# darksim33/Pyneapple

Measured on AMD Instinct MI355X. Metric: voxels/sec (pixelwise triexp LM & 250-bin NNLS) at 1/2/4/8 MI355X, higher is better.
Workload: dtype f64

## Files before the change

### pyneapple_amd/csrc/pnx_api.hip

```cpp
#include <hip/hip_runtime.h>

#include <cmath>
#include <cstdarg>
#include <cstdio>
#include <cstring>
#include <algorithm>
#include <atomic>
#include <chrono>
#include <condition_variable>
#include <cstdlib>
#include <functional>
#include <mutex>
#include <string>
#include <thread>
#include <vector>

#include "pnx_curvefit_f32_kernel.hpp"
#include "pnx_curvefit_kernel.hpp"
#include "pnx_grid.hpp"
#include "pnx_grid_args.hpp"
#include "pnx_grid_class.hpp"
#include "pnx_grid_posterior.hpp"
#include "pnx_grid_marginal.hpp"
#include "pnx_grid_mrf.hpp"
// ... 109 lines not shown

static void touch_pages(void *p, size_t bytes) {
    if (!p || !bytes) return;
    volatile char *c = (volatile char *)p;
    const uintptr_t a = (uintptr_t)p;
    c[0] = 0;
    for (size_t off = (4096 - (a & 4095)) & 4095; off < bytes; off += 4096) c[off] = 0;
}

int env_int(const char *name, int dflt, int lo, int hi) {
    const char *e = getenv(name);
    if (!e) return dflt;
    const long v = atol(e);
    return v < lo ? lo : (v > hi ? hi : (int)v);
}
const char *dev_getenv(const char *name) {
    static const bool enabled = [] {
        const char *e = getenv("PNX_ENABLE_TEST_HOOKS");
        return e && e[0] == '1' && e[1] == 0;
    }();
    return enabled ? getenv(name) : nullptr;
}
int dev_env_int(const char *name, int dflt, int lo, int hi) { return dev_getenv(name) ? env_int(name, dflt, lo, hi) : dflt; }

static std::atomic<int> g_host_calls(0);
struct HostCallGuard {
    int in_flight;
    HostCallGuard() : in_flight(g_host_calls.fetch_add(1) + 1) {}
    ~HostCallGuard() { g_host_calls.fetch_sub(1); }
    int touchers() const { return getenv("PNX_HOST_TOUCHERS") ? env_int("PNX_HOST_TOUCHERS", 2, 0, 8) : (in_flight >= 3 ? 0 : (in_flight == 2 ? 1 : 2)); }
    int out_threads() const { return getenv("PNX_STREAM_OUT_THREADS") ? env_int("PNX_STREAM_OUT_THREADS", 2, 1, 4) : (in_flight >= 4 ? 1 : 2); }
};

struct Carver {
    char *base = nullptr;
    size_t off = 0;
    void *take(size_t bytes) {
        void *p = base ? base + off : nullptr;
        off += (bytes + 255) & ~(size_t)255;
        return p;
    }
};

static int model_n_params(int model) {
    switch (model) {
    case PNX_MODEL_MONO: return 2;
    case PNX_MODEL_BI_REDUCED: return 3;
    case PNX_MODEL_BI_S0: return 4;
    case PNX_MODEL_BI_FULL: return 4;
    case PNX_MODEL_TRI_REDUCED: return 5;
    case PNX_MODEL_TRI_S0: return 6;
    case PNX_MODEL_TRI_FULL: return 6;
    }
    return -1;
}

typedef int (*launch_fn)(int, int, const CurvefitArgs *, int, void *);
static launch_fn g_launch[7] = {pnx_launch_curvefit_m0, pnx_launch_curvefit_m1, pnx_launch_curvefit_m2,
                                pnx_launch_curvefit_m3, pnx_launch_curvefit_m4, pnx_launch_curvefit_m5,
                                pnx_launch_curvefit_m6};

struct StreamLaunch {
    StreamCtl *ctl = nullptr;
    unsigned int *host_flags = nullptr;
    int granule_shift = 0;
    unsigned int spins = 0;
    int phase = 0;
};

static int curvefit_device(const pnx_curvefit_opts *o, int64_t n_vox, const double *b, const double *y_d,
                           const double *p0, const double *lo, const double *hi, const double *fixed, double *popt_d,
                           double *pcov_d, int8_t *status_d, int32_t *nfev_d, double *cost_d, DeviceInfo *dev,
                           hipStream_t stream, const StreamLaunch *sl = nullptr, const int32_t *order = nullptr) {
    CurvefitArgs a;
    memset(&a, 0, sizeof(a));
    if (sl) {
        a.ctl = sl->ctl;
        a.host_flags = sl->host_flags;
        a.granule_shift = sl->granule_shift;
        a.stream_spins = sl->spins;
        a.phase = sl->phase;
    }
    a.team = dev_env_int("PNX_CF_TEAM", 1, 0, 1);
    a.order = sl ? nullptr : order;
    a.y = y_d;
    a.popt = popt_d;
    a.pcov = pcov_d;
    a.status = status_d;
    a.nfev = nfev_d;
    a.cost = cost_d;
    a.n_vox = n_vox;
    a.n_b = o->n_b;
    a.per_voxel = o->per_voxel_p0_bounds;
    a.fixed_per_voxel = o->fixed_per_voxel;
    a.max_nfev = o->max_nfev > 0 ? o->max_nfev : 100 * o->n_free;
    a.n_fixed = o->n_fixed;
    a.t1_mode = o->t1_mode;
    a.tr = o->tr;
    a.tm = o->tm;
    a.ftol = o->ftol;
    a.xtol = o->xtol;
    a.gtol = o->gtol;
    for (int k = 0; k < o->n_free; ++k) a.free_idx[k] = o->free_idx[k];
    for (int k = 0; k < o->n_fixed; ++k) a.fixed_idx[k] = o->fixed_idx[k];
    for (int i = 0; i < o->n_b; ++i) a.b[i] = b[i];
    a.absolute_sigma = o->absolute_sigma != 0;
    a.use_sigma = o->sigma != nullptr;
    if (o->sigma)
        for (int i = 0; i < o->n_b; ++i) a.w[i] = 1.0 / o->sigma[i];
    if (o->per_voxel_p0_bounds) {
        a.p0 = p0;
        a.lo = lo;
        a.hi = hi;
    } else {
        for (int k = 0; k < o->n_free; ++k) {
            a.p0s[k] = p0[k];
            a.los[k] = lo[k];
            a.his[k] = hi[k];
        }
    }
    if (o->n_fixed) {
        if (o->fixed_per_voxel)
            a.fixed = fixed;
        else
            for (int k = 0; k < o->n_fixed; ++k) a.fixeds[k] = fixed[k];
    }
    if (a.phase != 2) {
        a.queue = next_queue(dev);
        PNX_HIP(hipMemsetAsync(a.queue, 0, sizeof(unsigned long long), stream));
    }
    return g_launch[o->model](o->n_free, o->jac_mode, &a, dev->cus, (void *)stream);
}

static int check_curvefit_opts(const pnx_curvefit_opts *o) {
    if (!o) return set_error(PNX_ERR_INVALID, "opts is NULL");
    int n_all = model_n_params(o->model);
    if (n_all < 0) return set_error(PNX_ERR_INVALID, "unknown model %d", o->model);
    if (o->t1_mode < 0 || o->t1_mode > 2) return set_error(PNX_ERR_INVALID, "t1_mode %d", o->t1_mode);
    if (o->t1_mode) n_all += 1;
    if (o->n_b < 1 || o->n_b > PNX_MAX_BVALUES) return set_error(PNX_ERR_INVALID, "n_b=%d out of range [1,%d]", o->n_b, PNX_MAX_BVALUES);
    if (o->n_free < 1 || o->n_fixed < 0 || o->n_free + o->n_fixed != n_all)
        return set_error(PNX_ERR_INVALID, "n_free=%d + n_fixed=%d != %d parameters of model %d", o->n_free, o->n_fixed, n_all, o->model);
    bool seen[PNX_MAX_PARAMS] = {false};
    for (int k = 0; k < o->n_free; ++k) {
        const int j = o->free_idx[k];
        if (j < 0 || j >= n_all || seen[j] || (k && j <= o->free_idx[k - 1]))
            return set_error(PNX_ERR_INVALID, "free_idx must be ascending, unique positions in [0,%d)", n_all);
        seen[j] = true;
    }
    for (int k = 0; k < o->n_fixed; ++k) {
        const int j = o->fixed_idx[k];
        if (j < 0 || j >= n_all || seen[j]) return set_error(PNX_ERR_INVALID, "fixed_idx overlaps free_idx or is out of range");
        seen[j] = true;
    }
    if (o->jac_mode != PNX_JAC_FD && o->jac_mode != PNX_JAC_ANALYTIC) return set_error(PNX_ERR_INVALID, "jac_mode %d", o->jac_mode);
    if (o->jac_mode == PNX_JAC_FD && o->n_fixed)
        return set_error(PNX_ERR_UNSUPPORTED,
                         "finite-difference Jacobian with fixed parameters: the reference uses the analytic Jacobian "
                         "there (curvefit.py:274-288); pass PNX_JAC_ANALYTIC");
    if (!(o->ftol >= 0) || !(o->xtol >= 0) || !(o->gtol >= 0)) return set_error(PNX_ERR_INVALID, "tolerances must be >= 0");
    return PNX_OK;
}

}

using namespace pnx;
// ... 2872 lines not shown
```

### pyneapple_amd/csrc/pnx_curvefit_kernel.hpp

```cpp
#pragma once
#include <hip/hip_runtime.h>
#include <stdint.h>

#include "pnx_trf_math.hpp"

namespace pnx {

constexpr int kWave = 64;
constexpr int kMaxB = 128;
constexpr int kMaxP = 8;
#ifdef PNX_ROW_BLK
template <int N> constexpr int row_blk() { return PNX_ROW_BLK; }
#else
template <int N> constexpr int row_blk() { return N >= 7 ? 2 : (N >= 5 ? 4 : 8); }
#endif
constexpr double kEps = TrfTraits<double>::eps;
constexpr double kSqrtEps = 1.4901161193847656e-08;
template <bool B> struct BoolC {
    static constexpr bool value = B;
};
typedef __attribute__((address_space(3))) void lds_void;

struct StreamCtl {
    unsigned long long ready;
    unsigned int abort;
    unsigned int timed_out;
    unsigned int done[1];
};

struct CurvefitArgs {
    const double *y;
    const double *p0;
    const double *lo;
    const double *hi;
    const double *fixed;
    double *popt;
    double *pcov;
    int8_t *status;
    int32_t *nfev;
    double *cost;
    unsigned long long *queue;
    const int32_t *order;
    StreamCtl *ctl;
    unsigned int *host_flags;
    int granule_shift;
    unsigned int stream_spins;
    int phase;
    int team;
    long long n_vox;
    int n_b;
    int per_voxel;
    int fixed_per_voxel;
    int max_nfev;
    int n_fixed;
    int t1_mode;
    double tr, tm;
    double ftol, xtol, gtol;
    double p0s[kMaxP], los[kMaxP], his[kMaxP], fixeds[kMaxP];
    int free_idx[kMaxP];
    int fixed_idx[kMaxP];
    int use_sigma;
    int absolute_sigma;
    double b[kMaxB];
    double w[kMaxB];
};

template <int MODEL> struct Model;

template <> struct Model<0> {
    static constexpr int NALL = 2, NC = 1;
    __device__ static constexpr int dpos(int c) { return 1; }
    __device__ static double signal(const double *p, const double *E) { return p[0] * E[0]; }
    __device__ static void jac(const double *p, const double *E, double x, double *r) {
        r[0] = E[0];
        r[1] = -x * p[0] * E[0];
    }
};
template <> struct Model<1> {
    static constexpr int NALL = 3, NC = 2;
    __device__ static constexpr int dpos(int c) { return c == 0 ? 1 : 2; }
    __device__ static double signal(const double *p, const double *E) { return p[0] * E[0] + (1 - p[0]) * E[1]; }
    __device__ static void jac(const double *p, const double *E, double x, double *r) {
        r[0] = E[0] - E[1];
        r[1] = -x * p[0] * E[0];
        r[2] = -x * (1 - p[0]) * E[1];
    }
};
template <> struct Model<2> {
    static constexpr int NALL = 4, NC = 2;
    __device__ static constexpr int dpos(int c) { return c == 0 ? 1 : 2; }
    __device__ static double signal(const double *p, const double *E) {
        return p[3] * (p[0] * E[0] + (1 - p[0]) * E[1]);
    }
    __device__ static void jac(const double *p, const double *E, double x, double *r) {
        r[0] = p[3] * (E[0] - E[1]);
        r[1] = -x * p[3] * p[0] * E[0];
        r[2] = -x * p[3] * (1 - p[0]) * E[1];
        r[3] = p[0] * E[0] + (1 - p[0]) * E[1];
    }
};
template <> struct Model<3> {
    static constexpr int NALL = 4, NC = 2;
    __device__ static constexpr int dpos(int c) { return c == 0 ? 1 : 3; }
    __device__ static double signal(const double *p, const double *E) { return p[0] * E[0] + p[2] * E[1]; }
    __device__ static void jac(const double *p, const double *E, double x, double *r) {
        r[0] = E[0];
        r[1] = -x * p[0] * E[0];
        r[2] = E[1];
        r[3] = -x * p[2] * E[1];
    }
};
template <> struct Model<4> {
    static constexpr int NALL = 5, NC = 3;
    __device__ static constexpr int dpos(int c) { return c == 0 ? 1 : (c == 1 ? 3 : 4); }
    __device__ static double signal(const double *p, const double *E) {
        return p[0] * E[0] + p[2] * E[1] + (1 - p[0] - p[2]) * E[2];
    }
    __device__ static void jac(const double *p, const double *E, double x, double *r) {
        const double f3 = 1 - p[0] - p[2];
        r[0] = E[0] - E[2];
        r[1] = -x * p[0] * E[0];
        r[2] = E[1] - E[2];
        r[3] = -x * p[2] * E[1];
        r[4] = -x * f3 * E[2];
    }
};
template <> struct Model<5> {
    static constexpr int NALL = 6, NC = 3;
    __device__ static constexpr int dpos(int c) { return c == 0 ? 1 : (c == 1 ? 3 : 4); }
    __device__ static double signal(const double *p, const double *E) {
        return p[5] * (p[0] * E[0] + p[2] * E[1] + (1 - p[0] - p[2]) * E[2]);
    }
    __device__ static void jac(const double *p, const double *E, double x, double *r) {
        const double f3 = 1 - p[0] - p[2], S0 = p[5];
        r[0] = S0 * (E[0] - E[2]);
        r[1] = -x * S0 * p[0] * E[0];
        r[2] = S0 * (E[1] - E[2]);
        r[3] = -x * S0 * p[2] * E[1];
        r[4] = -x * S0 * f3 * E[2];
        r[5] = p[0] * E[0] + p[2] * E[1] + f3 * E[2];
    }
};
template <> struct Model<6> {
    static constexpr int NALL = 6, NC = 3;
    __device__ static constexpr int dpos(int c) { return c == 0 ? 1 : (c == 1 ? 3 : 5); }
    __device__ static double signal(const double *p, const double *E) {
        return p[0] * E[0] + p[2] * E[1] + p[4] * E[2];
    }
    __device__ static void jac(const double *p, const double *E, double x, double *r) {
        r[0] = E[0];
        r[1] = -x * p[0] * E[0];
        r[2] = E[1];
        r[3] = -x * p[2] * E[1];
        r[4] = E[2];
        r[5] = -x * p[4] * E[2];
    }
};

template <int MODEL> __host__ __device__ constexpr int colperm(int k) {
    constexpr int P[7][6] = {{0, 1, 2, 3, 4, 5}, {2, 0, 1, 3, 4, 5}, {2, 0, 1, 3, 4, 5}, {3, 1, 2, 0, 4, 5},
                             {4, 3, 0, 2, 1, 5}, {4, 3, 0, 2, 1, 5}, {5, 3, 1, 4, 2, 0}};
    return P[MODEL][k];
}

template <int MODEL> __device__ constexpr int comp_of_param(int j) {
    for (int c = 0; c < Model<MODEL>::NC; ++c)
        if (Model<MODEL>::dpos(c) == j) return c;
    return -1;
}

#ifndef PNX_CF_FAST_EXP
#define PNX_CF_FAST_EXP 1
#endif
#ifndef PNX_CF_HINTS
#define PNX_CF_HINTS 1
#endif
#if PNX_CF_HINTS
#define PNX_LIKELY(x) __builtin_expect(!!(x), 1)
#else
#define PNX_LIKELY(x) (x)
#endif
__device__ inline double exp_fast(double x) {
#if PNX_CF_FAST_EXP
    const double k = __builtin_rint(x * 1.4426950408889634);
    double r = fma(k, -0.6931471805599453, x);
    r = fma(k, -2.3190468138462996e-17, r);
    const double r2 = r * r;
    double qe = 2.7630903490112654e-07;
    qe = fma(qe, r2, 2.480149103909504e-05);
    qe = fma(qe, r2, 0.0013888888945916382);
    qe = fma(qe, r2, 0.041666666666519754);
    qe = fma(qe, r2, 0.5000000000000012);
    double qo = 2.502232256764614e-08;
    qo = fma(qo, r2, 2.755751454582531e-06);
    qo = fma(qo, r2, 0.00019841269589115522);
    qo = fma(qo, r2, 0.008333333333455043);
    qo = fma(qo, r2, 0.16666666666666477);
    const double q = fma(r, qo, qe);
    return ldexp(fma(r, fma(r, q, 1.0), 1.0), __double2int_rz(k));
#else
    return exp(x);
#endif
}

__device__ inline double lane_bcast(double v, int src) {
    const unsigned long long u = __builtin_bit_cast(unsigned long long, v);
    const unsigned int lo = __builtin_amdgcn_readlane((int)(unsigned int)u, src), hi = __builtin_amdgcn_readlane((int)(unsigned int)(u >> 32), src);
    return __builtin_bit_cast(double, ((unsigned long long)hi << 32) | lo);
}

enum LaneState : int { ST_IDLE = 0, ST_INIT = 1, ST_RUN = 2, ST_FINAL = 3 };

template <int N> struct Park {
    static constexpr int NR = N * (N + 1) / 2;
    static constexpr bool kParkV = (N <= 5);
    static constexpr int NV = kParkV ? N * N : 0;
    __host__ __device__ static constexpr int per_wave(int tile_rows) { return kWave * (tile_rows + NR + NV); }
    __host__ __device__ static constexpr int per_wave_f64(int n_b) { return kWave * (((n_b + 1) & ~1) + NR + NV); }
};

#ifndef PNX_CF_WAVES_PER_SIMD
#define PNX_CF_WAVES_PER_SIMD 1
#endif
#ifndef PNX_CF_BLOCK_WAVES
#define PNX_CF_BLOCK_WAVES 4
#endif
template <int MODEL, int N, bool FD, bool PV, bool T1, bool STREAM = false>
__global__ void __launch_bounds__(64 * PNX_CF_BLOCK_WAVES, PNX_CF_WAVES_PER_SIMD) curvefit_kernel(const CurvefitArgs A) {
    using M = Model<MODEL>;
    using PK = Park<N>;
    constexpr int NALL = M::NALL;
    constexpr int NP = NALL + (T1 ? 1 : 0);
    constexpr int NC = M::NC;
    constexpr bool HASFIXED = (N != NP);
    static_assert(!(FD && HASFIXED), "finite-difference mode is only built without fixed parameters");
    auto CP = [](int k) constexpr { return (HASFIXED || k >= NALL) ? k : colperm<MODEL>(k); };

    extern __shared__ double smem[];
    const int n_b = A.n_b;
    double *bsh = smem;
    const int lane = threadIdx.x & (kWave - 1);
    const int wave = threadIdx.x / kWave;
    const bool use_w = A.use_sigma != 0;
    const double *wsh = smem + kMaxB;
    double *ytile = smem + (use_w ? 2 * kMaxB : kMaxB) + (size_t)wave * PK::per_wave_f64(n_b);
    double *ysh = ytile + 2 * lane;
    double *rpark = ytile + (size_t)((n_b + 1) & ~1) * kWave + lane;
    double *vpark = rpark + (size_t)PK::NR * kWave;
    for (int i = threadIdx.x; i < n_b; i += blockDim.x) bsh[i] = A.b[i];
    if (use_w)
        for (int i = threadIdx.x; i < n_b; i += blockDim.x) smem[kMaxB + i] = A.w[i];
    double bmax = 0;
    for (int i = 0; i < n_b; ++i) {
        const double ab = fabs(A.b[i]);
        bmax = (ab < INFINITY) ? fmax(bmax, ab) : INFINITY;
    }
    __syncthreads();
    const bool dma_ok = ((reinterpret_cast<uintptr_t>(A.y) & 7) == 0);

    int state = ST_IDLE;
    long long vox = -1;
    unsigned long long ready_seen = 0;
    int pub = 0;
    auto publish = [&](bool all) {
        const int n_gran = (int)((A.n_vox + (1ll << A.granule_shift) - 1) >> A.granule_shift);
        int upto = pub;
        while (upto < n_gran && (all || !__ballot(state != ST_IDLE && (vox >> A.granule_shift) <= upto))) ++upto;
        if (upto == pub) return;
        __builtin_amdgcn_fence(__ATOMIC_RELEASE, "");
        const unsigned int n_waves = gridDim.x * (blockDim.x / kWave);
        if ((threadIdx.x & (kWave - 1)) == __ffsll((unsigned long long)__ballot(1)) - 1) {
            for (int g = pub; g < upto; ++g) {
                const unsigned int old = __hip_atomic_fetch_add(&A.ctl->done[g], 1u, __ATOMIC_ACQ_REL, __HIP_MEMORY_SCOPE_SYSTEM);
                if (old + 1 == n_waves) __hip_atomic_store(&A.host_flags[g], 1u, __ATOMIC_RELEASE, __HIP_MEMORY_SCOPE_SYSTEM);
            }
        }
        pub = upto;
    };
    double x[N], lb[N], ub[N];
    double pfull[NP];
    double g[N];
    double s[N], uf[N], R2[N][N], d[N], g_h[N];
    double Vreg[PK::kParkV ? 1 : N][PK::kParkV ? 1 : N];
    double smax = 0, smin = 0, theta = 0;
    double cost = 0, Delta = 0, alpha = 0;
    int nfev = 0, term = -99;
    bool first = false;
    double xn[N], step_h_norm = 0, step_norm = 0, predicted = 0;
    if (!PV) {
#pragma unroll
        for (int k = 0; k < N; ++k) {
            lb[k] = A.los[k];
            ub[k] = A.his[k];
        }
    }

#ifdef PNX_CF_STAMP
    unsigned long long seg[9] = {0, 0, 0, 0, 0, 0, 0, 0, 0}, act[9] = {0, 0, 0, 0, 0, 0, 0, 0, 0}, cnt[9] = {0, 0, 0, 0, 0, 0, 0, 0, 0};
    unsigned long long tl = __builtin_amdgcn_s_memtime();
    bool cf_in_team = false;
#define CFSTAMP(k) do { __builtin_amdgcn_s_waitcnt(0); const unsigned long long t_ = __builtin_amdgcn_s_memtime(); if ((k) == 8 || !cf_in_team) { seg[k] += t_ - tl; tl = t_; } } while (0)
#define CFACT(k, cond) do { act[k] += __popcll(__ballot(cond)); cnt[k] += 1; } while (0)
#else
#define CFSTAMP(k) do {} while (0)
#define CFACT(k, cond) do {} while (0)
#endif
    auto refill = [&]() {
    while (state == ST_IDLE) {
        const unsigned long long idx = atomicAdd(A.queue, 1ULL);
        if (idx >= (unsigned long long)A.n_vox) break;
        if constexpr (STREAM) {
            if (idx >= ready_seen) {
                bool got = false;
                const unsigned int *abort_word = A.host_flags + ((A.n_vox + (1ll << A.granule_shift) - 1) >> A.granule_shift);
                for (unsigned int spins = 0; spins < A.stream_spins; ++spins) {
                    ready_seen = __hip_atomic_load(&A.ctl->ready, __ATOMIC_ACQUIRE, __HIP_MEMORY_SCOPE_SYSTEM);
                    if (idx < ready_seen) {
                        got = true;
                        break;
                    }
                    if ((spins & 15u) == 15u && __hip_atomic_load(abort_word, __ATOMIC_RELAXED, __HIP_MEMORY_SCOPE_SYSTEM)) break;
                    __builtin_amdgcn_s_sleep(127);
                }
                if (!got) {
                    if (!__hip_atomic_load(abort_word, __ATOMIC_RELAXED, __HIP_MEMORY_SCOPE_SYSTEM))
                        __hip_atomic_store(&A.ctl->timed_out, 1u, __ATOMIC_RELAXED, __HIP_MEMORY_SCOPE_SYSTEM);
                    break;
                }
            }
        }
        vox = (long long)idx;
        if constexpr (!STREAM) {
            if (A.order) vox = A.order[idx];
        }
        const double *yv = A.y + (size_t)vox * n_b;
        if (dma_ok) {
            const int pairs = n_b >> 1;
            for (int c = 0; c < pairs; ++c)
                __builtin_amdgcn_global_load_lds((const void *)(yv + 2 * c), (lds_void *)(ytile + c * 2 * kWave), 16, 0, 0);
            if (n_b & 1) {
                if (vox + 1 < A.n_vox)
                    __builtin_amdgcn_global_load_lds((const void *)(yv + n_b - 1), (lds_void *)(ytile + pairs * 2 * kWave), 16, 0, 0);
                else
                    ysh[pairs * 2 * kWave] = yv[n_b - 1];
            }
        } else {
            for (int i = 0; i < n_b; ++i) ysh[(i >> 1) * 2 * kWave + (i & 1)] = yv[i];
        }
        bool okb = true, okp = true;
        double p0v[N];
#pragma unroll
        for (int k = 0; k < N; ++k) {
            if (PV) {
                p0v[k] = A.p0[(size_t)k * A.n_vox + vox];
                lb[k] = A.lo[(size_t)k * A.n_vox + vox];
                ub[k] = A.hi[(size_t)k * A.n_vox + vox];
            } else
                p0v[k] = A.p0s[k];
            okb = okb && (lb[k] < ub[k]);
            okp = okp && (p0v[k] >= lb[k]) && (p0v[k] <= ub[k]);
        }
        if (HASFIXED) {
#pragma unroll
            for (int j = 0; j < NP; ++j) pfull[j] = 0;
            for (int f = 0; f < A.n_fixed; ++f) {
                const double fv = A.fixed_per_voxel ? A.fixed[(size_t)f * A.n_vox + vox] : A.fixeds[f];
#pragma unroll
                for (int j = 0; j < NP; ++j)
                    if (A.fixed_idx[f] == j) pfull[j] = fv;
            }
        }
        if (!okb || !okp) {
            const int st = !okb ? -1 : -3;
#pragma unroll
            for (int k = 0; k < N; ++k) A.popt[(size_t)k * A.n_vox + vox] = p0v[k];
            if (A.status) A.status[vox] = (int8_t)st;
            if (A.nfev) A.nfev[vox] = 0;
            if (A.cost) A.cost[vox] = NAN;
            continue;
        }
#pragma unroll
        for (int k = 0; k < N; ++k) xn[k] = strictly_feasible_r(p0v[k], lb[k], ub[k]);
        state = ST_INIT;
        nfev = 0;
        term = -99;
        alpha = 0.0;
    }
    };
    refill();
    if constexpr (STREAM) {
        if (!__ballot(state != ST_IDLE)) publish(true);
    }
    auto iterate = [&](auto team_c, const int owner) __attribute__((always_inline)) {
        constexpr bool TM = decltype(team_c)::value;
        asm volatile("s_waitcnt vmcnt(0)" ::: "memory");
        CFSTAMP(0);
        CFACT(1, true);

        double Rn[N][N], qn[N], gn[N], cost_new = 0;
        bool finite_f = true, yfinite = true;
        {
            if constexpr (TM) {
#pragma unroll
                for (int k = 0; k < N; ++k) {
                    xn[k] = lane_bcast(xn[k], owner);
                    if (PV) {
                        lb[k] = lane_bcast(lb[k], owner);
                        ub[k] = lane_bcast(ub[k], owner);
                    }
                }
                if (HASFIXED) {
#pragma unroll
                    for (int j = 0; j < NP; ++j) pfull[j] = lane_bcast(pfull[j], owner);
                }
            }
            double pe[NP];
            if (HASFIXED) {
#pragma unroll
                for (int j = 0; j < NP; ++j) {
                    pe[j] = pfull[j];
#pragma unroll
                    for (int k = 0; k < N; ++k)
                        if (A.free_idx[k] == j) pe[j] = xn[k];
                }
            } else {
#pragma unroll
                for (int j = 0; j < NP; ++j) pe[j] = xn[j];
            }
            double dxv[N];
            if (FD) {
#pragma unroll
                for (int k = 0; k < N; ++k) {
                    const double sign = (xn[k] >= 0) ? 1.0 : -1.0;
                    double h = kSqrtEps * sign * fmax(1.0, fabs(xn[k]));
                    const double lower_dist = xn[k] - lb[k], upper_dist = ub[k] - xn[k];
                    const double xx = xn[k] + h;
                    const bool violated = (xx < lb[k]) || (xx > ub[k]);
                    const bool fitting = fabs(h) <= fmax(lower_dist, upper_dist);
                    if (violated && fitting) h = -h;
                    if (!fitting) h = (upper_dist >= lower_dist) ? upper_dist : -lower_dist;
                    dxv[k] = (xn[k] + h) - xn[k];
                }
            }
            double A1 = 1.0, eTM = 1.0, fac = 1.0, dfac = 0.0;
            if (T1) {
                const bool steam = A.t1_mode == 2;
                const double T1v = pe[T1 ? NALL : 0];
                const double eTR = exp(-A.tr / T1v);
                A1 = 1 - eTR;
                eTM = steam ? exp(-A.tm / T1v) : 1.0;
                fac = A1 * eTM;
                dfac = steam ? eTM / (T1v * T1v) * (-A.tr * eTR + A.tm * A1) : (-eTR * A.tr / (T1v * T1v));
                if (FD) {
                    const double dx = dxv[N - 1];
                    const double T2 = T1v + dx;
                    const double fac2 = (1 - exp(-A.tr / T2)) * (steam ? exp(-A.tm / T2) : 1.0);
                    dfac = (fac2 - fac) / dx;
                }
            }
#pragma unroll
            for (int i = 0; i < N; ++i) {
                qn[i] = 0;
                gn[i] = 0;
#pragma unroll
                for (int j = 0; j < N; ++j) Rn[i][j] = 0;
            }
            constexpr int kRowBlk = row_blk<N>();
            static_assert(kRowBlk % 2 == 0, "a block reads its signal values as [pair][lane][2] pairs");
            auto row_eval = [&](auto fastgz_c, auto usew_c, auto tail_c, const int ii, const double bb, const double yi, double &r0_out,
                                double (&jr)[N]) __attribute__((always_inline)) {
                constexpr bool FASTGZ = decltype(fastgz_c)::value, USEW = decltype(usew_c)::value, TAIL = decltype(tail_c)::value;
                const double nb = -bb;
                double E[NC];
#pragma unroll
                for (int c = 0; c < NC; ++c) E[c] = exp_fast(nb * pe[M::dpos(c)]);
                const double base = M::signal(pe, E);
                double r0 = (T1 ? base * A1 * eTM : base) - yi;
                {
                    double ja[NP];
// ... 47 lines not shown
                const double rr = live ? r0 : 0.0;
                finite_f = finite_f && isfinite(rr);
                cost_new += rr * rr;
#pragma unroll
                for (int k = 0; k < N; ++k) {
                    const double jk = live ? jr[k] : 0.0;
                    gn[k] += jk * rr;
                }
#pragma unroll
                for (int k = 0; k < N; ++k) brow[k] = live ? jr[CP(k)] : 0.0;
                brow[N] = rr;
            };
            auto row_block = [&](auto fastgz_c, auto usew_c, auto tail_c, const int i0) __attribute__((always_inline)) {
                constexpr bool TAIL = decltype(tail_c)::value;
                double blk[kRowBlk][N + 1];
                double bv[TAIL ? 1 : kRowBlk], yv[TAIL ? 1 : kRowBlk];
                if constexpr (!TAIL) {
#pragma unroll
                    for (int r = 0; r < kRowBlk; r += 2) {
                        const double2 b2 = *reinterpret_cast<const double2 *>(bsh + i0 + r);
                        const double2 y2 = *reinterpret_cast<const double2 *>(ysh + (size_t)(i0 + r) * kWave);
                        bv[r] = b2.x;
                        bv[r + 1] = b2.y;
                        yv[r] = y2.x;
                        yv[r + 1] = y2.y;
                    }
                }
#pragma unroll
                for (int r = 0; r < kRowBlk; ++r) {
                    const bool live = !TAIL || (i0 + r < n_b);
                    const int ii = live ? i0 + r : 0;
                    const double bb = TAIL ? bsh[ii] : bv[TAIL ? 0 : r];
                    const double yi = TAIL ? ysh[(ii >> 1) * 2 * kWave + (ii & 1)] : yv[TAIL ? 0 : r];
                    yfinite = yfinite && isfinite(yi);
                    double r0, jr[N];
                    row_eval(fastgz_c, usew_c, tail_c, ii, bb, yi, r0, jr);
                    row_consume(blk[r], live, r0, jr);
                }
                CFSTAMP(1);
                qr_merge<N, kRowBlk>(Rn, qn, blk);
                CFSTAMP(6);
            };
            auto row_loop = [&](auto fastgz_c, auto usew_c) __attribute__((always_inline)) {
                int i0 = 0;
                for (; i0 + kRowBlk <= n_b; i0 += kRowBlk) row_block(fastgz_c, usew_c, BoolC<false>{}, i0);
                if (i0 < n_b) row_block(BoolC<false>{}, BoolC<false>{}, BoolC<true>{}, i0);
            };
            constexpr bool kOneLoop = (N >= 6);
            bool gz_cubic = FD && PNX_CF_FAST_EXP && !kOneLoop;
            if (FD && PNX_CF_FAST_EXP && !kOneLoop) {
                bool in_range = true;
#pragma unroll
                for (int k = 0; k < NALL; ++k)
                    if (comp_of_param<MODEL>(k) >= 0) in_range = in_range && (fabs(bmax * dxv[k]) < 2e-4);
                gz_cubic = __ballot(!in_range) == 0;
            }
            if constexpr (TM) {
                static_assert(N + 1 <= 8 && 2 * kWave == kMaxB, "a team row is 8 doubles; two rows per lane cover every n_b");
                double *trow = ytile + (owner < kWave / 2 ? kWave : 0);
                const double *yown = ytile + 2 * owner;
                bool ybad = false;
                __builtin_amdgcn_fence(__ATOMIC_ACQ_REL, "wavefront");
#pragma unroll
                for (int h = 0; h < kMaxB / kWave; ++h) {
                    if (h * kWave < n_b) {
                        const int i = lane + h * kWave;
                        const bool live = i < n_b;
                        const int ii = live ? i : 0;
                        const double yi = yown[(ii >> 1) * 2 * kWave + (ii & 1)];
                        ybad = ybad || !isfinite(yi);
                        double r0, jr[N];
                        row_eval(BoolC<false>{}, BoolC<false>{}, BoolC<true>{}, ii, bsh[ii], yi, r0, jr);
                        if (live) {
                            double *tr = trow + (i >> 1) * 2 * kWave + (i & 1) * 8;
#pragma unroll
                            for (int k = 0; k < N; ++k) tr[k] = jr[k];
                            tr[N] = r0;
                        }
                    }
                }
                yfinite = __ballot(ybad) == 0;
                __builtin_amdgcn_fence(__ATOMIC_ACQ_REL, "wavefront");
                __builtin_amdgcn_wave_barrier();
                for (int i0 = 0; i0 < n_b; i0 += kRowBlk) {
                    double blk[kRowBlk][N + 1];
#pragma unroll
                    for (int r = 0; r < kRowBlk; ++r) {
                        const bool live = i0 + r < n_b;
                        const int ii = live ? i0 + r : 0;
                        const double *tr = trow + (ii >> 1) * 2 * kWave + (ii & 1) * 8;
                        double jr[N];
#pragma unroll
                        for (int k = 0; k < N; ++k) jr[k] = tr[k];
                        row_consume(blk[r], live, tr[N], jr);
                    }
                    qr_merge<N, kRowBlk>(Rn, qn, blk);
                }
            } else if constexpr (kOneLoop) {
                for (int i0 = 0; i0 < n_b; i0 += kRowBlk) row_block(BoolC<false>{}, BoolC<false>{}, BoolC<true>{}, i0);
            } else if (PNX_LIKELY(!use_w && (gz_cubic || !FD))) {
                if constexpr (FD && PNX_CF_FAST_EXP)
                    row_loop(BoolC<true>{}, BoolC<false>{});
                else
                    row_loop(BoolC<false>{}, BoolC<false>{});
            } else if (use_w) {
                row_loop(BoolC<false>{}, BoolC<true>{});
            } else {
                if constexpr (FD) row_loop(BoolC<false>{}, BoolC<false>{});
            }
            cost_new *= 0.5;
        }

        CFSTAMP(1);
        if constexpr (TM) {
            if (state == ST_IDLE) return;
        }
        bool accepted = false;
        int final_status = 0;
        if (state == ST_INIT) {
            if (!finite_f) {
                final_status = yfinite ? -4 : -2;
                cost = NAN;
                nfev = 0;
                state = ST_FINAL;
            } else {
                accepted = true;
                nfev = 1;
                first = true;
                state = ST_RUN;
            }
        } else {
            nfev += 1;
            if (!finite_f) {
                Delta = 0.25 * step_h_norm;
            } else {
                const double actual = cost - cost_new;
                double ratio;
                if (predicted > 0)
                    ratio = actual / predicted;
                else if (predicted == 0 && actual == 0)
                    ratio = 1;
                else
                    ratio = 0;
                double Delta_new = Delta;
                if (ratio < 0.25)
                    Delta_new = 0.25 * step_h_norm;
                else if (ratio > 0.75 && step_h_norm > 0.95 * Delta)
                    Delta_new = Delta * 2.0;
                const bool ftol_ok = (actual < A.ftol * cost) && (ratio > 0.25);
                const bool xtol_ok = step_norm < A.xtol * (A.xtol + normn<N>(x));
                if (ftol_ok && xtol_ok)
                    term = 4;
                else if (ftol_ok)
                    term = 2;
                else if (xtol_ok)
                    term = 3;
                if (term == -99) {
                    alpha *= Delta / Delta_new;
                    Delta = Delta_new;
                }
                accepted = actual > 0;
            }
        }
        if (accepted) {
#pragma unroll
            for (int i = 0; i < N; ++i) {
                x[i] = xn[i];
                g[i] = gn[i];
            }
            cost = cost_new;
            int t = 0;
#pragma unroll
            for (int i = 0; i < N; ++i)
#pragma unroll
                for (int j = i; j < N; ++j) rpark[(t++) * kWave] = Rn[i][j];
        }

        double v[N], dv[N], g_norm = 0;
        if (state == ST_RUN && (accepted || term != -99 || nfev >= A.max_nfev)) {
#pragma unroll
            for (int i = 0; i < N; ++i) {
                v[i] = 1.0;
                dv[i] = 0.0;
                if (g[i] < 0 && isfinite(ub[i])) {
                    v[i] = ub[i] - x[i];
                    dv[i] = -1;
                }
                if (g[i] > 0 && isfinite(lb[i])) {
                    v[i] = x[i] - lb[i];
                    dv[i] = 1;
                }
                g_norm = fmax(g_norm, fabs(g[i] * v[i]));
            }
            if (first) {
                double t = 0;
#pragma unroll
                for (int i = 0; i < N; ++i) {
                    const double q = x[i] / sqrt(v[i]);
                    t += q * q;
                }
                Delta = sqrt(t);
                if (Delta == 0) Delta = 1.0;
                first = false;
            }
            if (g_norm < A.gtol) term = 1;
            if (term != -99 || nfev >= A.max_nfev) {
                final_status = (term == -99) ? 0 : term;
                state = ST_FINAL;
            }
        }

        CFSTAMP(2);
        CFACT(3, state == ST_FINAL);
        if (state == ST_FINAL) {
            const bool ok = final_status > 0;
#pragma unroll
            for (int k = 0; k < N; ++k) {
                const double pk = ok ? x[k] : (PV ? A.p0[(size_t)k * A.n_vox + vox] : A.p0s[k]);
                A.popt[(size_t)k * A.n_vox + vox] = pk;
            }
            if (A.status) A.status[vox] = (int8_t)final_status;
            if (A.nfev) A.nfev[vox] = nfev;
            if (A.cost) A.cost[vox] = cost;
            if (A.pcov && ok) {
                double *pc = A.pcov + (size_t)vox * N * N;
#pragma unroll
                for (int t = 0; t < PK::NR; ++t) pc[t] = rpark[t * kWave];
            }
            state = ST_IDLE;
        }
        CFACT(0, state == ST_IDLE);
        if constexpr (STREAM) {
            const bool any_idle = __ballot(state == ST_IDLE) != 0;
            if (state == ST_IDLE) refill();
            if (any_idle) publish(false);
        } else if constexpr (!TM) {
            if (state == ST_IDLE) refill();
        }

        CFSTAMP(3);
        CFACT(4, state == ST_RUN && accepted);
        CFACT(5, state == ST_RUN);
        if (state == ST_RUN) {
            if (accepted) {
                double diag_h[N];
#pragma unroll
                for (int i = 0; i < N; ++i) {
                    d[i] = sqrt(v[i]);
                    diag_h[i] = g[i] * dv[i];
                    g_h[i] = d[i] * g[i];
                }
                double q2[N];
                double blk[N][N + 1];
#pragma unroll
                for (int i = 0; i < N; ++i) {
                    q2[i] = qn[i];
#pragma unroll
                    for (int j = 0; j < N; ++j) {
                        R2[i][j] = (j >= i) ? Rn[i][j] * d[CP(j)] : 0.0;
                        blk[i][j] = (i == j) ? sqrt(diag_h[CP(i)]) : 0.0;
                    }
                    blk[i][N] = 0.0;
                }
                qr_merge<N, N>(R2, q2, blk);
                double W[N][N], Vw[N][N];
#pragma unroll
                for (int i = 0; i < N; ++i)
#pragma unroll
                    for (int j = 0; j < N; ++j) W[i][j] = (i >= j) ? R2[j][i] : 0.0;
                jacobi_svd<N>(W, Vw);
                smax = 0;
                smin = INFINITY;
#pragma unroll
                for (int k = 0; k < N; ++k) {
                    double nn = 0, dq = 0;
#pragma unroll
                    for (int i = 0; i < N; ++i) {
                        nn += W[i][k] * W[i][k];
                        dq += Vw[i][k] * q2[i];
                    }
                    double inv = 0.0;
                    if (nn > 0) nn = fast_sqrt_rsqrt(nn, &inv);
                    s[k] = nn;
                    uf[k] = dq;
#pragma unroll
                    for (int i = 0; i < N; ++i) {
                        if (PK::kParkV)
                            vpark[(i * N + k) * kWave] = W[i][k] * inv;
                        else
                            Vreg[PK::kParkV ? 0 : i][PK::kParkV ? 0 : k] = W[i][k] * inv;
                    }
                    smax = fmax(smax, nn);
                    smin = fmin(smin, nn);
                }
                theta = fmax(0.995, 1 - g_norm);
            }
            CFSTAMP(4);
            double V[N][N];
#pragma unroll
            for (int i = 0; i < N; ++i)
#pragma unroll
                for (int k = 0; k < N; ++k)
                    V[i][k] = PK::kParkV ? vpark[(i * N + k) * kWave] : Vreg[PK::kParkV ? 0 : i][PK::kParkV ? 0 : k];
            double xP[N], lbP[N], ubP[N], dP[N], ghP[N];
#pragma unroll
            for (int i = 0; i < N; ++i) {
                xP[i] = x[CP(i)];
                lbP[i] = lb[CP(i)];
                ubP[i] = ub[CP(i)];
                dP[i] = d[CP(i)];
                ghP[i] = g_h[CP(i)];
            }
            double p_h[N], p[N], step[N], step_h[N];
            alpha = solve_lsq_trust_region<N>(n_b, uf, s, V, smax, smin, Delta, alpha, p_h);
#pragma unroll
            for (int i = 0; i < N; ++i) p[i] = dP[i] * p_h[i];
            predicted = select_step<N>(xP, R2, ghP, p, p_h, dP, Delta, lbP, ubP, theta, step, step_h);
#pragma unroll
            for (int i = 0; i < N; ++i) xn[CP(i)] = strictly_feasible0(xP[i] + step[i], lbP[i], ubP[i]);
            step_h_norm = normn<N>(step_h);
            step_norm = normn<N>(step);
            CFSTAMP(5);
        }
    };
    constexpr bool kTeam = !STREAM && N <= 5;
    constexpr int kTeamMax = 1;
    for (;;) {
        CFSTAMP(7);
        if (state == ST_IDLE) break;
        if constexpr (kTeam) {
            if (!PNX_LIKELY(__popcll(__ballot(1)) > kTeamMax || !A.team)) break;
        }
        iterate(BoolC<false>{}, 0);
    }
    if constexpr (kTeam) {
#ifdef PNX_CF_STAMP
        cf_in_team = true;
#endif
        for (;;) {
            const unsigned long long livem = __ballot(state != ST_IDLE);
            if (!livem) break;
            iterate(BoolC<true>{}, __ffsll(livem) - 1);
            CFSTAMP(8);
            CFACT(8, true);
        }
    }
#ifdef PNX_CF_STAMP
    if (threadIdx.x == 0 && blockIdx.x == 3)
        printf("CFSTAMP refill=%llu pass_rows=%llu pass_qr_merge=%llu D+Blight=%llu final=%llu Bheavy=%llu C=%llu loop=%llu team=%llu | iters=%llu team_iters=%llu idle_at_top=%.2f final=%.2f Bheavy=%.2f run=%.2f\n",
               seg[0], seg[1], seg[6], seg[2], seg[3], seg[4], seg[5], seg[7], seg[8], cnt[1], cnt[8], (double)act[0] / cnt[0], (double)act[3] / cnt[3],
               (double)act[4] / cnt[4], (double)act[5] / cnt[5]);
#endif
}

struct ColPerm {
    int p[kMaxP];
};

template <int N>
__global__ void __launch_bounds__(256) pcov_kernel(double *pcov, const int8_t *status, const double *cost,
                                                   long long n_vox, int n_b, const ColPerm cp, int absolute_sigma) {
    const long long vox = (long long)blockIdx.x * blockDim.x + threadIdx.x;
    if (vox >= n_vox) return;
    double *pc = pcov + (size_t)vox * N * N;
    if (status[vox] <= 0) {
#pragma unroll
        for (int k = 0; k < N * N; ++k) pc[k] = NAN;
        return;
    }
    double W[N][N], Vw[N][N];
    {
        int t = 0;
#pragma unroll
        for (int i = 0; i < N; ++i)
#pragma unroll
            for (int j = 0; j < N; ++j) W[i][j] = 0.0;
#pragma unroll
        for (int i = 0; i < N; ++i)
#pragma unroll
            for (int j = i; j < N; ++j) W[j][i] = pc[t++];
    }
    jacobi_svd<N>(W, Vw);
    double s2[N], sm = 0;
#pragma unroll
    for (int k = 0; k < N; ++k) {
        double nn = 0;
#pragma unroll
        for (int i = 0; i < N; ++i) nn += W[i][k] * W[i][k];
        s2[k] = nn;
        sm = fmax(sm, nn);
    }
    const double thr = kEps * (n_b > N ? n_b : N) * sqrt(sm);
    const bool dof = absolute_sigma || n_b > N;
    const double s_sq = absolute_sigma ? 1.0 : (dof ? 2.0 * cost[vox] / (double)(n_b - N) : 0.0);
    double wgt[N];
#pragma unroll
    for (int k = 0; k < N; ++k) wgt[k] = (sqrt(s2[k]) > thr) ? 1.0 / (s2[k] * s2[k]) : 0.0;
    bool bad = false;
    double out[N][N];
#pragma unroll
    for (int i = 0; i < N; ++i)
#pragma unroll
        for (int j = 0; j < N; ++j) {
            double a = 0;
#pragma unroll
            for (int k = 0; k < N; ++k) a += W[i][k] * W[j][k] * wgt[k];
            out[i][j] = a;
            bad = bad || isnan(a);
        }
#pragma unroll
    for (int i = 0; i < N; ++i)
#pragma unroll
        for (int j = 0; j < N; ++j) pc[cp.p[i] * N + cp.p[j]] = (bad || !dof) ? INFINITY : out[i][j] * s_sq;
}

}
```

### pyneapple_amd/csrc/pnx_trf_math.hpp

```cpp
#pragma once
#include <hip/hip_runtime.h>

#include <type_traits>

namespace pnx {

template <typename T> struct TrfTraits;

template <> struct TrfTraits<double> {
    static constexpr double eps = 2.220446049250313e-16;
    static constexpr double jacobi_skip = 1.0e-30, jacobi_rotated = 1.0e-16;
    static constexpr double rstep = 1e-10;
    static constexpr double alpha_floor = 0.001, phi_rtol = 0.01;
    __device__ static inline double rcp(double x) {
        double r = __builtin_amdgcn_rcp(x);
        r = fma(fma(-x, r, 1.0), r, r);
        r = fma(fma(-x, r, 1.0), r, r);
        return r;
    }
    __device__ static inline double sqrt_rsqrt(double x, double *rs) {
        double y = __builtin_amdgcn_rsq(x);
        double g = x * y, h = 0.5 * y;
        double r = fma(-h, g, 0.5);
        g = fma(g, r, g);
        h = fma(h, r, h);
        r = fma(-h, g, 0.5);
        g = fma(g, r, g);
        h = fma(h, r, h);
        *rs = h + h;
        return g;
    }
};

template <> struct TrfTraits<float> {
    static constexpr float eps = 1.1920929e-07f;
    static constexpr float jacobi_skip = 1.0e-13f, jacobi_rotated = 1.0e-7f;
    static constexpr float rstep = 8.0f * eps;
    static constexpr float alpha_floor = 0.001f, phi_rtol = 0.01f;
    __device__ static inline float rcp(float x) {
        float r = __builtin_amdgcn_rcpf(x);
        return fmaf(fmaf(-x, r, 1.0f), r, r);
    }
    __device__ static inline float sqrt_rsqrt(float x, float *rs) {
        const float y = __builtin_amdgcn_rsqf(x);
        float g = x * y, h = 0.5f * y;
        const float r = fmaf(-h, g, 0.5f);
        g = fmaf(g, r, g);
        h = fmaf(h, r, h);
        *rs = h + h;
        return g;
    }
};

template <typename T> __device__ inline T fast_rcp(T x) { return TrfTraits<T>::rcp(x); }
template <typename T> __device__ inline T fast_sqrt_rsqrt(T x, T *rs) { return TrfTraits<T>::sqrt_rsqrt(x, rs); }

template <int N, typename T> __device__ inline T dotn(const T *a, const T *b) {
    T s = 0;
#pragma unroll
    for (int i = 0; i < N; ++i) s += a[i] * b[i];
    return s;
}
template <int N, typename T> __device__ inline T normn(const T *a) { return sqrt(dotn<N>(a, a)); }

template <int N, int RB, typename T> __device__ inline void qr_merge(T (&R)[N][N], T (&q)[N], T (&blk)[RB][N + 1]) {
#pragma unroll
    for (int k = 0; k < N; ++k) {
        T sig = 0;
#pragma unroll
        for (int r = 0; r < RB; ++r) sig += blk[r][k] * blk[r][k];
        if (sig > 0) {
            const T alpha = R[k][k];
            T rs;
            const T nrm = fast_sqrt_rsqrt(alpha * alpha + sig, &rs);
            const T beta = alpha <= 0 ? nrm : -nrm;
            const T v0 = alpha - beta;
            const T inv_v0 = copysign(fast_rcp(fabs(v0)), v0);
            const T tau = -v0 * (alpha <= 0 ? rs : -rs);
#pragma unroll
            for (int r = 0; r < RB; ++r) blk[r][k] *= inv_v0;
            R[k][k] = beta;
#pragma unroll
            for (int j = k + 1; j <= N; ++j) {
                T w = (j < N) ? R[k][j] : q[k];
#pragma unroll
                for (int r = 0; r < RB; ++r) w += blk[r][k] * blk[r][j];
                w *= tau;
                if (j < N)
                    R[k][j] -= w;
                else
                    q[k] -= w;
#pragma unroll
                for (int r = 0; r < RB; ++r) blk[r][j] -= w * blk[r][k];
            }
        }
    }
}

template <int N, typename T> __device__ inline void jacobi_svd(T (&W)[N][N], T (&V)[N][N]) {
    using Tr = TrfTraits<T>;
#pragma unroll
    for (int i = 0; i < N; ++i)
#pragma unroll
        for (int j = 0; j < N; ++j) V[i][j] = (i == j) ? T(1) : T(0);
    if (N == 1) return;
    for (int sweep = 0; sweep < 30; ++sweep) {
        bool rotated = false;
#pragma unroll
        for (int p = 0; p < N - 1; ++p) {
#pragma unroll
            for (int q = p + 1; q < N; ++q) {
                T a = 0, b = 0, g = 0;
#pragma unroll
                for (int i = 0; i < N; ++i) {
                    a += W[i][p] * W[i][p];
                    b += W[i][q] * W[i][q];
                    g += W[i][p] * W[i][q];
                }
                const T g2 = g * g, ab = a * b;
                if (g2 > Tr::jacobi_skip * ab) {
                    rotated = rotated || (g2 >= Tr::jacobi_rotated * ab);
                    const T num = b - a, den = T(2) * g;
                    T rs;
                    const T hyp = fast_sqrt_rsqrt(num * num + den * den, &rs);
                    T t = fabs(den) * fast_rcp(fabs(num) + hyp);
                    t = ((num < 0) != (den < 0)) ? -t : t;
                    T c;
                    (void)fast_sqrt_rsqrt(T(1) + t * t, &c);
                    const T s = c * t;
#pragma unroll
                    for (int i = 0; i < N; ++i) {
                        const T wp = W[i][p], wq = W[i][q];
                        W[i][p] = c * wp - s * wq;
                        W[i][q] = s * wp + c * wq;
                        const T vp = V[i][p], vq = V[i][q];
                        V[i][p] = c * vp - s * vq;
                        V[i][q] = s * vp + c * vq;
                    }
                }
            }
        }
        if (!rotated) break;
    }
}

template <typename T> __device__ inline T strictly_feasible0(T x, T lb, T ub) {
    if (x <= lb) x = nextafter(lb, ub);
    if (x >= ub) x = nextafter(ub, lb);
    if (x < lb || x > ub) x = T(0.5) * (lb + ub);
    return x;
}
template <typename T> __device__ inline T strictly_feasible_r(T x, T lb, T ub) {
    const T rstep = TrfTraits<T>::rstep;
    const T lower_dist = x - lb, upper_dist = ub - x;
    const T lt = rstep * fmax(T(1), fabs(lb)), ut = rstep * fmax(T(1), fabs(ub));
    int active = 0;
    if (isfinite(lb) && lower_dist <= fmin(upper_dist, lt)) active = -1;
    if (isfinite(ub) && upper_dist <= fmin(lower_dist, ut)) active = 1;
    if (active == -1) x = lb + lt;
    if (active == 1) x = ub - ut;
    if (x < lb || x > ub) x = T(0.5) * (lb + ub);
    return x;
}

template <int N, typename T>
__device__ inline T step_size_to_bound(const T *x, const T *s, const T *lb, const T *ub, int *hits) {
    T steps[N];
    T mn = T(INFINITY);
#pragma unroll
    for (int i = 0; i < N; ++i) {
        const T num = (s[i] > 0) ? (ub[i] - x[i]) : (lb[i] - x[i]);
        steps[i] = (s[i] != 0) ? num / s[i] : T(INFINITY);
        mn = fmin(mn, steps[i]);
    }
    if (hits) {
#pragma unroll
        for (int i = 0; i < N; ++i) hits[i] = (steps[i] == mn) ? ((s[i] > 0) - (s[i] < 0)) : 0;
    }
    return mn;
// ... 223 lines not shown
```

Before: 137.4 million.

## Pipeline team-mode QR merge across lanes with a DPP systolic skew

In team mode, where a whole wave iterates one lone voxel, each lane now builds its own row block and the QR merge runs as a systolic wavefront. Column factors pass lane to lane with a DPP shift, replacing the serial per-block qr_merge loop run redundantly by every lane. qr_merge is refactored into a reusable qr_col_step helper. The path is on by default through PNX_CF_TEAM_MERGE and the old path stays behind the flag. It also adds team-segment timing stamps and a lone-voxel profiling script. One oddity: an extra loop still calls team_block over all blocks (presumably for the cost and gradient side effects), which adds redundant work.

```diff
diff --git a/profiles/curvefit_lone_voxel.py b/profiles/curvefit_lone_voxel.py
--- /dev/null
+++ b/profiles/curvefit_lone_voxel.py
@@ -0,0 +1,53 @@
+#!/usr/bin/env python
+import os
+import sys
+
+os.environ["PNX_ENABLE_TEST_HOOKS"] = "1"
+sys.path.insert(0, os.path.dirname(os.path.dirname(os.path.abspath(__file__))))
+import numpy as np
+import torch
+
+from pyneapple_amd import _build, api, synth
+
+args = sys.argv[1:]
+reps = int(args.pop(0)) if args and args[0].isdigit() else 8
+hooks = args or ["PNX_CF_TEAM_MERGE=0", "PNX_CF_TEAM_MERGE=1"]
+dev = torch.device("cuda", 0)
+n_b = 32
+_, p0, lo, hi = synth.shared_arrays("tri_reduced")
+opts = api.make_opts("tri_reduced", n_b, per_voxel=False, max_nfev=250, ftol=1e-8, jac="fd")
+
+
+def launch(y, timed=False):
+    m = y.shape[0]
+    popt = torch.empty((5, m), dtype=torch.float64, device=dev)
+    status = torch.empty((m,), dtype=torch.int8, device=dev)
+    nfev = torch.empty((m,), dtype=torch.int32, device=dev)
+    cost = torch.empty((m,), dtype=torch.float64, device=dev)
+    e0, e1 = torch.cuda.Event(enable_timing=True), torch.cuda.Event(enable_timing=True)
+    e0.record()
+    api.curvefit_device(opts, m, b, y, p0, lo, hi, None, popt, None, status, nfev, cost, 0, torch.cuda.current_stream().cuda_stream)
+    e1.record()
+    torch.cuda.synchronize()
+    return nfev.cpu().numpy(), e0.elapsed_time(e1)
+
+
+b, pool = synth.make_torch("tri_reduced", 1 << 16, n_b, dev, sigma=0.05)
+nf, _ = launch(pool)
+run = np.where(nf < 250, nf, -1)
+longest = int(run.argmax())
+quick = np.argsort(nf, kind="stable")[:64]
+y = torch.cat([pool[torch.from_numpy(quick).to(dev)], pool[longest:longest + 1]]).contiguous()
+print(f"# curvefit source id {_build.source_id('curvefit')}; lib {os.path.basename(os.environ.get('PNX_LIB', 'product'))}")
+print(f"longest voxel {longest} nfev {nf[longest]} quick max {nf[quick].max()}")
+for _ in range(2):
+    for h in hooks:
+        k, v = h.split("=")
+        os.environ[k] = v
+        ms = []
+        for _ in range(reps):
+            n65, t = launch(y)
+            ms.append(t)
+        del os.environ[k]
+        ms = np.sort(ms[1:])
+        print(f"{h} nfev_last={n65[64]} ms min/med/max = {ms[0]:.4f} {np.median(ms):.4f} {ms[-1]:.4f}  us/eval = {1e3 * np.median(ms) / n65[64]:.2f}")
diff --git a/pyneapple_amd/csrc/pnx_api.hip b/pyneapple_amd/csrc/pnx_api.hip
--- a/pyneapple_amd/csrc/pnx_api.hip
+++ b/pyneapple_amd/csrc/pnx_api.hip
@@ -215,6 +215,7 @@
         a.phase = sl->phase;
     }
     a.team = dev_env_int("PNX_CF_TEAM", 1, 0, 1);
+    a.team_merge = dev_env_int("PNX_CF_TEAM_MERGE", 1, 0, 1);
     a.order = sl ? nullptr : order;
     a.y = y_d;
     a.popt = popt_d;
diff --git a/pyneapple_amd/csrc/pnx_curvefit_kernel.hpp b/pyneapple_amd/csrc/pnx_curvefit_kernel.hpp
--- a/pyneapple_amd/csrc/pnx_curvefit_kernel.hpp
+++ b/pyneapple_amd/csrc/pnx_curvefit_kernel.hpp
@@ -47,6 +47,7 @@
     unsigned int stream_spins;
     int phase;
     int team;
+    int team_merge;
     long long n_vox;
     int n_b;
     int per_voxel;
@@ -209,6 +210,14 @@
     return __builtin_bit_cast(double, ((unsigned long long)hi << 32) | lo);
 }
 
+__device__ inline double lane_from_below(double v) {
+    const unsigned long long u = __builtin_bit_cast(unsigned long long, v);
+    constexpr int kWaveShr1 = 0x138;
+    const unsigned int lo = __builtin_amdgcn_update_dpp(0, (int)(unsigned int)u, kWaveShr1, 0xf, 0xf, false),
+                       hi = __builtin_amdgcn_update_dpp(0, (int)(unsigned int)(u >> 32), kWaveShr1, 0xf, 0xf, false);
+    return __builtin_bit_cast(double, ((unsigned long long)hi << 32) | lo);
+}
+
 enum LaneState : int { ST_IDLE = 0, ST_INIT = 1, ST_RUN = 2, ST_FINAL = 3 };
 
 template <int N> struct Park {
@@ -301,8 +310,12 @@
     bool cf_in_team = false;
 #define CFSTAMP(k) do { __builtin_amdgcn_s_waitcnt(0); const unsigned long long t_ = __builtin_amdgcn_s_memtime(); if ((k) == 8 || !cf_in_team) { seg[k] += t_ - tl; tl = t_; } } while (0)
 #define CFACT(k, cond) do { act[k] += __popcll(__ballot(cond)); cnt[k] += 1; } while (0)
+    unsigned long long tseg[7] = {0, 0, 0, 0, 0, 0, 0}, ttl = 0;
+    int cf_owner = -1;
+#define CFSTAMP_TEAM(k) do { if (cf_in_team) { __builtin_amdgcn_s_waitcnt(0); const unsigned long long t_ = __builtin_amdgcn_s_memtime(); tseg[k] += t_ - ttl; ttl = t_; } } while (0)
 #else
 #define CFSTAMP(k) do {} while (0)
+#define CFSTAMP_TEAM(k) do {} while (0)
 #define CFACT(k, cond) do {} while (0)
 #endif
     auto refill = [&]() {
@@ -395,6 +408,7 @@
         constexpr bool TM = decltype(team_c)::value;
         asm volatile("s_waitcnt vmcnt(0)" ::: "memory");
         CFSTAMP(0);
+        CFSTAMP_TEAM(0);
         CFACT(1, true);
 
         double Rn[N][N], qn[N], gn[N], cost_new = 0;
@@ -608,8 +622,8 @@
                 yfinite = __ballot(ybad) == 0;
                 __builtin_amdgcn_fence(__ATOMIC_ACQ_REL, "wavefront");
                 __builtin_amdgcn_wave_barrier();
-                for (int i0 = 0; i0 < n_b; i0 += kRowBlk) {
-                    double blk[kRowBlk][N + 1];
+                CFSTAMP_TEAM(1);
+                auto team_block = [&](double (&blk)[kRowBlk][N + 1], const int i0) __attribute__((always_inline)) {
 #pragma unroll
                     for (int r = 0; r < kRowBlk; ++r) {
                         const bool live = i0 + r < n_b;
@@ -620,8 +634,55 @@
                         for (int k = 0; k < N; ++k) jr[k] = tr[k];
                         row_consume(blk[r], live, tr[N], jr);
                     }
-                    qr_merge<N, kRowBlk>(Rn, qn, blk);
-                }
+                };
+                constexpr bool kTeamSkew = N >= 3;
+                bool skew = false;
+                if constexpr (kTeamSkew) skew = A.team_merge != 0;
+                if (!skew) {
+                    for (int i0 = 0; i0 < n_b; i0 += kRowBlk) {
+                        double blk[kRowBlk][N + 1];
+                        team_block(blk, i0);
+                        qr_merge<N, kRowBlk>(Rn, qn, blk);
+                    }
+                } else if constexpr (kTeamSkew) {
+                    const int n_blk = (n_b + kRowBlk - 1) / kRowBlk, last = n_blk - 1;
+                    double col[kRowBlk][N + 1], fac[N + 1];
+                    team_block(col, lane < n_blk ? lane * kRowBlk : n_b);
+                    finite_f = true;
+                    cost_new = 0;
+#pragma unroll
+                    for (int k = 0; k < N; ++k) gn[k] = 0;
+                    for (int i0 = 0; i0 < n_b; i0 += kRowBlk) {
+                        double blk[kRowBlk][N + 1];
+                        team_block(blk, i0);
+                    }
+#pragma unroll
+                    for (int i = 0; i <= N; ++i) fac[i] = 0;
+                    for (int t = 0; t < n_blk + N - 1; ++t) {
+#pragma unroll
+                        for (int i = 0; i <= N; ++i) fac[i] = lane_from_below(fac[i]);
+                        const int j = t - lane;
+                        if (lane < n_blk && j >= 0 && j < N) {
+                            qr_col_step<kRowBlk, N, double>([&](int i) -> double & { return fac[i]; },
+                                                            [&](int r, int i) -> double & { return col[r][i]; });
+#pragma unroll
+                            for (int r = 0; r < kRowBlk; ++r) {
+#pragma unroll
+                                for (int i = 0; i < N; ++i) col[r][i] = col[r][i + 1];
+                                col[r][N] = 0;
+                            }
+                        }
+#pragma unroll
+                        for (int jj = 0; jj < N; ++jj) {
+                            if (t - last == jj) {
+#pragma unroll
+                                for (int i = 0; i < N - jj; ++i) Rn[jj][jj + i] = lane_bcast(fac[i], last);
+                                qn[jj] = lane_bcast(fac[N - jj], last);
+                            }
+                        }
+                    }
+                }
+                CFSTAMP_TEAM(2);
             } else if constexpr (kOneLoop) {
                 for (int i0 = 0; i0 < n_b; i0 += kRowBlk) row_block(BoolC<false>{}, BoolC<false>{}, BoolC<true>{}, i0);
             } else if (PNX_LIKELY(!use_w && (gz_cubic || !FD))) {
@@ -765,6 +826,7 @@
         }
 
         CFSTAMP(3);
+        CFSTAMP_TEAM(3);
         CFACT(4, state == ST_RUN && accepted);
         CFACT(5, state == ST_RUN);
         if (state == ST_RUN) {
@@ -822,6 +884,7 @@
                 theta = fmax(0.995, 1 - g_norm);
             }
             CFSTAMP(4);
+            CFSTAMP_TEAM(4);
             double V[N][N];
 #pragma unroll
             for (int i = 0; i < N; ++i)
@@ -841,12 +904,14 @@
             alpha = solve_lsq_trust_region<N>(n_b, uf, s, V, smax, smin, Delta, alpha, p_h);
 #pragma unroll
             for (int i = 0; i < N; ++i) p[i] = dP[i] * p_h[i];
+            CFSTAMP_TEAM(5);
             predicted = select_step<N>(xP, R2, ghP, p, p_h, dP, Delta, lbP, ubP, theta, step, step_h);
 #pragma unroll
             for (int i = 0; i < N; ++i) xn[CP(i)] = strictly_feasible0(xP[i] + step[i], lbP[i], ubP[i]);
             step_h_norm = normn<N>(step_h);
             step_norm = normn<N>(step);
             CFSTAMP(5);
+            CFSTAMP_TEAM(6);
         }
     };
     constexpr bool kTeam = !STREAM && N <= 5;
@@ -862,10 +927,14 @@
     if constexpr (kTeam) {
 #ifdef PNX_CF_STAMP
         cf_in_team = true;
+        ttl = __builtin_amdgcn_s_memtime();
 #endif
         for (;;) {
             const unsigned long long livem = __ballot(state != ST_IDLE);
             if (!livem) break;
+#ifdef PNX_CF_STAMP
+            cf_owner = __ffsll(livem) - 1;
+#endif
             iterate(BoolC<true>{}, __ffsll(livem) - 1);
             CFSTAMP(8);
             CFACT(8, true);
@@ -876,6 +945,9 @@
         printf("CFSTAMP refill=%llu pass_rows=%llu pass_qr_merge=%llu D+Blight=%llu final=%llu Bheavy=%llu C=%llu loop=%llu team=%llu | iters=%llu team_iters=%llu idle_at_top=%.2f final=%.2f Bheavy=%.2f run=%.2f\n",
                seg[0], seg[1], seg[6], seg[2], seg[3], seg[4], seg[5], seg[7], seg[8], cnt[1], cnt[8], (double)act[0] / cnt[0], (double)act[3] / cnt[3],
                (double)act[4] / cnt[4], (double)act[5] / cnt[5]);
+    if (cnt[8] >= 50 && lane == cf_owner)
+        printf("CFSTAMP_TEAM block=%d wave=%d team_iters=%llu loop=%llu rows=%llu merge=%llu D+Blight+final=%llu Bheavy=%llu C_head=%llu select_step=%llu\n",
+               (int)blockIdx.x, wave, cnt[8], tseg[0], tseg[1], tseg[2], tseg[3], tseg[4], tseg[5], tseg[6]);
 #endif
 }
 
diff --git a/pyneapple_amd/csrc/pnx_trf_math.hpp b/pyneapple_amd/csrc/pnx_trf_math.hpp
--- a/pyneapple_amd/csrc/pnx_trf_math.hpp
+++ b/pyneapple_amd/csrc/pnx_trf_math.hpp
@@ -63,38 +63,44 @@
 }
 template <int N, typename T> __device__ inline T normn(const T *a) { return sqrt(dotn<N>(a, a)); }
 
+template <int RB, int NT, typename T, typename RowAt, typename ColAt> __device__ inline void qr_col_step(RowAt row, ColAt col) {
+    T sig = 0;
+#pragma unroll
+    for (int r = 0; r < RB; ++r) sig += col(r, 0) * col(r, 0);
+    if (sig > 0) {
+        const T alpha = row(0);
+        T rs;
+        const T nrm = fast_sqrt_rsqrt(alpha * alpha + sig, &rs);
+        const T beta = alpha <= 0 ? nrm : -nrm;
+        const T v0 = alpha - beta;
+        const T inv_v0 = copysign(fast_rcp(fabs(v0)), v0);
+        const T tau = -v0 * (alpha <= 0 ? rs : -rs);
+#pragma unroll
+        for (int r = 0; r < RB; ++r) col(r, 0) *= inv_v0;
+        row(0) = beta;
+#pragma unroll
+        for (int i = 1; i <= NT; ++i) {
+            T w = row(i);
+#pragma unroll
+            for (int r = 0; r < RB; ++r) w += col(r, 0) * col(r, i);
+            w *= tau;
+            row(i) -= w;
+#pragma unroll
+            for (int r = 0; r < RB; ++r) col(r, i) -= w * col(r, 0);
+        }
+    }
+}
+
+template <int N, int RB, int K, typename T> __device__ inline void qr_merge_from(T (&R)[N][N], T (&q)[N], T (&blk)[RB][N + 1]) {
+    if constexpr (K < N) {
+        qr_col_step<RB, N - K, T>([&](int i) -> T & { return (K + i < N) ? R[K][K + i] : q[K]; },
+                                  [&](int r, int i) -> T & { return blk[r][K + i]; });
+        qr_merge_from<N, RB, K + 1>(R, q, blk);
+    }
+}
+
 template <int N, int RB, typename T> __device__ inline void qr_merge(T (&R)[N][N], T (&q)[N], T (&blk)[RB][N + 1]) {
-#pragma unroll
-    for (int k = 0; k < N; ++k) {
-        T sig = 0;
-#pragma unroll
-        for (int r = 0; r < RB; ++r) sig += blk[r][k] * blk[r][k];
-        if (sig > 0) {
-            const T alpha = R[k][k];
-            T rs;
-            const T nrm = fast_sqrt_rsqrt(alpha * alpha + sig, &rs);
-            const T beta = alpha <= 0 ? nrm : -nrm;
-            const T v0 = alpha - beta;
-            const T inv_v0 = copysign(fast_rcp(fabs(v0)), v0);
-            const T tau = -v0 * (alpha <= 0 ? rs : -rs);
-#pragma unroll
-            for (int r = 0; r < RB; ++r) blk[r][k] *= inv_v0;
-            R[k][k] = beta;
-#pragma unroll
-            for (int j = k + 1; j <= N; ++j) {
-                T w = (j < N) ? R[k][j] : q[k];
-#pragma unroll
-                for (int r = 0; r < RB; ++r) w += blk[r][k] * blk[r][j];
-                w *= tau;
-                if (j < N)
-                    R[k][j] -= w;
-                else
-                    q[k] -= w;
-#pragma unroll
-                for (int r = 0; r < RB; ++r) blk[r][j] -= w * blk[r][k];
-            }
-        }
-    }
+    qr_merge_from<N, RB, 0>(R, q, blk);
 }
 
 template <int N, typename T> __device__ inline void jacobi_svd(T (&W)[N][N], T (&V)[N][N]) {
```

Measured after the change: 137.9 million, median of 6. No clear change (+0.3%).
